# A-Kokolis/Hermes

Measured on AMD Instinct MI355X. Metric: replicated KVS ops/s (reads+writes committed), higher is better.
Workload: dtype u8

## Files before the change

hermes_amd/csrc/hkv_batch_dev.h:

```cpp
#pragma once
#include <hip/hip_runtime.h>

#include <type_traits>

#include "hkv_exec.h"
#include "hkv_internal.h"
#include "hkv_table_dev.h"

namespace hkv {

constexpr uint32_t kNone = 0xFFFFFFFFu;
enum : uint8_t { kStDone = 0, kStCommit = 1, kStPend = 2, kStDefer = 3 };
enum { kCtrFbM = 1, kCtrFbL = 2, kCtrDefer = 3 };

struct BatchArgs {
    uint8_t *elems;
    const int32_t *counts;
    const int32_t *offsets;
    const uint8_t *index;
    uint8_t *log;
    uint8_t *rw;
    int32_t *ns_idx;
    unsigned long long *fw;
    unsigned long long *fx, *fy;
    unsigned long long *ft;
    uint32_t fw_mask;
    uint32_t *ent;
    uint8_t *st;
    uint32_t *pf;
    uint8_t *shadow;
    unsigned long long *mem;
    uint32_t *fbl;
    uint32_t *ctr;
    unsigned int *error_flags;
    Geometry g;
    int64_t n;
    int64_t rw_stride;
    int32_t stride;
    int32_t esz;
    int32_t type;
    uint32_t rtag0;
    uint8_t ltag;
    int32_t rounds;
    int32_t inv_direct;
    int32_t ack_direct;
    uint8_t g_membership;
    uint8_t w_ack_init;
    int32_t *node_suspected;
    int32_t n_batches;
    const uint8_t *host_src;
    uint8_t *host_dst;
    uint8_t *dev_region;
    uint64_t region_bytes;
    uint32_t *done_flag;
    uint32_t done_value;
    unsigned long long *prof;
    const SmallBatch *hdr;
    uint8_t *state_out;
    const uint8_t *opc;
    const uint8_t *patch;
    uint16_t *fk;
    uint64_t *hx;
    uint8_t *rws;
    const uint8_t *rwo;
    int32_t n_rows, skip_row;
    int64_t row_stride;
    int32_t dbg;
    int32_t check_unique;
    uint8_t *ack_out;
    uint32_t ack_out_size;
    uint8_t *line;
};

enum class Engine : uint8_t {
    kSmall,
    kLocalDirect,
    kRows,
    kUniqueLds64,
    kUniqueLdsBig,
    kUniqueInPlace,
    kValsOnePass,
    kRoundsAckDirect,
    kRoundsInvDirect,
    kRoundsSlab,
    kRoundsInPlace,
};
enum class Patches : uint8_t {
    kNone,
    kApplyFirst,
    kByEngine,
    kInResolve,
};
constexpr uint32_t kPirMaxValue = 320;
constexpr uint32_t kWaveWordsMaxValue = 8 * 62;
static_assert(kPirMaxValue <= kWaveWordsMaxValue, "wave_value_copies_n ignores VCopy::fill: handle it there first");
struct BatchPlan {
    int refuse;
    Engine engine;
    Patches patches;
    int sv;
    int rmax, ch;
    int slab_threads;
    int64_t lookup_head;
    bool big;
    bool mixed;
    bool inv_direct, ack_direct;
    bool ack_out;
    bool state_out, opc;
    bool fk;
    bool rw_mirrors;
    bool node_suspected;
    bool il;
    bool inline_instance;
};

int launch_small(const BatchArgs &a, const BatchPlan &p, hipStream_t s);
int launch_local(const BatchArgs &a, const BatchPlan &p, hipStream_t s);

template <class F>
inline void with_sv(int sv, F &&f)
{
    if (sv == 31) f(std::integral_constant<int, 31>{});
    else if (sv == 287) f(std::integral_constant<int, 287>{});
    else f(std::integral_constant<int, 0>{});
}
template <class F>
inline void with_bool(bool b, F &&f)
{
    if (b) f(std::true_type{});
    else f(std::false_type{});
}

__device__ __forceinline__ Ctx make_ctx(const BatchArgs &a)
{
    Ctx c;
    c.g = a.g;
    c.g_membership = a.g_membership;
    c.w_ack_init = a.w_ack_init;
    c.rw = nullptr;
    c.rws = nullptr;
    c.rw_done = nullptr;
    c.vc = nullptr;
    return c;
}

__device__ __forceinline__ uint64_t phys_of(const BatchArgs &a, uint32_t e) { return (uint64_t)e * a.g.entry_unit; }
__device__ __forceinline__ uint8_t *entry_of(const BatchArgs &a, uint32_t e) { return a.log + phys_of(a, e); }

struct __attribute__((aligned(8))) U64x2 {
    uint64_t a, b;
};

template <int TYPE>
__device__ __forceinline__ uint8_t absorbing_state()
{
    return TYPE == kVals ? kValid : kWrite;
}

template <int TYPE>
__device__ __forceinline__ Meta after_first(const BatchArgs &a, const Meta &m0, uint32_t f, int f_is_put)
{
    Meta m1 = m0;
    m_set_state(m1, absorbing_state<TYPE>());
    if (TYPE != kLocal || a.g.skew == 0) return m1;
    uint8_t foc = f_is_put ? (uint8_t)kOpPut : a.elems[(int64_t)f * a.esz + 8];
    if (a.hx && !f_is_put) {
        const uint64_t pb = *reinterpret_cast<const uint64_t *>(a.patch + (int64_t)f * 16 + 8);
        if ((pb >> 48) & 0xFFu) foc = (uint8_t)pb;
    }
    if (foc != kOpGet) {
        m1.ver += 2;
        m_set_cid(m1, (uint8_t)a.g.machine_id);
    } else {
        m_set_state(m1, kReplay);
    }
    return m1;
}

__device__ __forceinline__ int32_t batch_of(const BatchArgs &a, int64_t i, int64_t &start)
{
    if (!a.offsets) {
        const int32_t b = (int32_t)(i / a.stride);
        start = (int64_t)b * a.stride;
        return b;
    }
    int lo = 0, hi = a.n_batches - 1;
    while (lo < hi) {
        const int mid = (lo + hi + 1) >> 1;
        if (a.offsets[mid] <= i) lo = mid; else hi = mid - 1;
    }
    start = a.offsets[lo];
    return lo;
}

__device__ __forceinline__ void elem_at(const BatchArgs &a, uint32_t i, uint8_t *&x, uint8_t &idx, Ctx &c)
{
    c.rw = nullptr;
    c.rws = nullptr;
    idx = 0;
    if (a.rw || !a.offsets) {
        int64_t start;
        const int32_t b = batch_of(a, i, start);
        idx = (uint8_t)(i - start);
        c.rw = a.rw ? a.rw + (int64_t)b * a.rw_stride : nullptr;
        c.rws = a.rws ? a.rws + (int64_t)b * (a.rw_stride / a.g.op_size) : nullptr;
        c.rwo = a.rwo ? a.rwo + (int64_t)b * (a.rw_stride / a.g.op_size) : nullptr;
    }
    x = a.elems + (int64_t)i * a.esz;
}

__device__ __forceinline__ void note_state(const BatchArgs &a, int64_t i, const uint8_t *x)
{
    if (a.state_out) a.state_out[i] = x[9];
}

__device__ __forceinline__ uint32_t fw_index(const BatchArgs &a, uint64_t phys)
{
    return (uint32_t)(((phys >> 6) * 0x9E3779B1ull) & a.fw_mask);
}
__device__ __forceinline__ unsigned long long *fw_of(const BatchArgs &a, uint32_t e) { return a.fw + fw_index(a, phys_of(a, e)); }

__device__ __forceinline__ uint32_t first_cand(unsigned long long f, uint32_t rtag)
{
    return (uint32_t)(f >> 32) == ~rtag ? (uint32_t)f : kNone;
}

__device__ __forceinline__ void offer(unsigned long long *f, uint32_t rtag, uint32_t i)
{
    const unsigned long long v = ((unsigned long long)(~rtag) << 32) | i;
    if (v < __hip_atomic_load(f, __ATOMIC_RELAXED, __HIP_MEMORY_SCOPE_AGENT)) atomicMin(f, v);
}

__device__ __forceinline__ uint8_t *shadow_of(const BatchArgs &a, uint32_t i)
{
    return a.shadow + (size_t)i * a.g.entry_size;
}

__device__ __forceinline__ void copy_entry(uint8_t *dst, const uint8_t *src, uint32_t bytes)
{
    struct __attribute__((aligned(8))) W16 {
        uint64_t a, b;
    };
    uint32_t o = 0;
    for (; o + 16 <= bytes; o += 16) *reinterpret_cast<W16 *>(dst + o) = *reinterpret_cast<const W16 *>(src + o);
    if (o < bytes) *reinterpret_cast<uint64_t *>(dst + o) = *reinterpret_cast<const uint64_t *>(src + o);
}

template <int TYPE, int SV>
__device__ __forceinline__ void apply_to_shadow(const BatchArgs &a, uint8_t *x, uint32_t i, const uint8_t *src)
{
    uint8_t *sh = shadow_of(a, i);
    Meta m;
    meta_load(src, m);
    if (SV == 31) {
        const uint4 *s4 = reinterpret_cast<const uint4 *>(src);
        uint4 *d4 = reinterpret_cast<uint4 *>(sh);
        const uint4 w0 = s4[0], w1 = s4[1], w2 = s4[2], w3 = s4[3];
        d4[0] = w0;
        d4[1] = w1;
        d4[2] = w2;
        d4[3] = w3;
    } else {
        copy_entry(sh, src, a.g.entry_size);
    }
    Ctx c = make_ctx(a);
    uint8_t *xg;
    uint8_t idx;
    elem_at(a, i, xg, idx, c);
    if (x) dispatch<SV>(TYPE, x, sh, idx, m, c);
    else dispatch<SV>(TYPE, xg, sh, idx, m, c);
    meta_store(sh, m);
}

__device__ __forceinline__ bool patch_valid(uint64_t pb) { return ((pb >> 48) & 0xFFu) != 0; }

__device__ __forceinline__ bool in_count(const BatchArgs &a, uint32_t i)
{
    if (!a.counts) return true;
    const uint32_t b = i / (uint32_t)a.stride;
    return (int32_t)(i - b * (uint32_t)a.stride) < a.counts[b];
}

__device__ __forceinline__ uint64_t line_key_meta(const uint4 &ln, Meta &m)
{
    const uint64_t ek = (uint64_t)(uint32_t)__shfl((int)ln.z, 0, 4) | ((uint64_t)(uint32_t)__shfl((int)ln.w, 0, 4) << 32);
    m.w4 = (uint32_t)__shfl((int)ln.x, 1, 4);
    m.w5 = (uint32_t)__shfl((int)ln.y, 1, 4);
    m.ver = (uint32_t)__shfl((int)ln.z, 1, 4);
    const uint32_t w7 = (uint32_t)__shfl((int)ln.w, 1, 4);
    const uint32_t b32 = (uint32_t)__shfl((int)ln.x, 2, 4) & 0xFFu;
    m.llw_cid = (uint8_t)w7;
    m.llw_ver = (w7 >> 8) | (b32 << 24);
    return ek;
}

constexpr int kLookupPair = 2;
template <int P = kLookupPair, bool IL = false, bool F = false>
__device__ __forceinline__ void lookup_core(const BatchArgs &a, const uint64_t *key, const bool *probe, int q,
                                            int gbase, bool *ok, uint64_t *phys, uint4 *ln, unsigned long long *fwv,
                                            uint8_t **home, bool *inl)
{
    uint4 v[P], ev[P];
#pragma unroll
    for (int k = 0; k < P; ++k) {
        if (IL) {
            const uint4 *l = line_words(a.line, bucket_of(a.g, key[k]));
            v[k] = probe[k] ? l[q] : make_uint4(0u, 0u, 0u, 0u);
            ev[k] = probe[k] ? l[4 + q] : make_uint4(0u, 0u, 0u, 0u);
        } else {
            v[k] = probe[k] ? bucket_words(a.index, bucket_of(a.g, key[k]))[q] : make_uint4(0u, 0u, 0u, 0u);
        }
    }
    bool il[P];
#pragma unroll
    for (int k = 0; k < P; ++k) {
        const uint64_t s0 = u64_of(v[k].x, v[k].y), s1 = u64_of(v[k].z, v[k].w);
        const uint32_t tag = key_tag(key[k]);
        const bool mt0 = probe[k] && (s0 & 1u) && ((uint32_t)(s0 >> 1) & 0x7FFFFFu) == tag;
        const bool mt1 = probe[k] && (s1 & 1u) && ((uint32_t)(s1 >> 1) & 0x7FFFFFu) == tag;
        const uint32_t g0 = (uint32_t)(__ballot(mt0) >> gbase) & 0xFu;
        const uint32_t g1 = (uint32_t)(__ballot(mt1) >> gbase) & 0xFu;
        uint32_t o = 0;
#pragma unroll
        for (int l = 0; l < 4; ++l) o |= ((g0 >> l) & 1u) << (2 * l) | ((g1 >> l) & 1u) << (2 * l + 1);
        const int first = o ? __ffs(o) - 1 : 0;
        const uint64_t raw = group_slot_word(slot_off_raw(s0), slot_off_raw(s1), first), off = off_of<IL>(raw);
        ok[k] = probe[k] && o && in_log_window(a.g, off);
        phys[k] = off & a.g.log_mask;
        il[k] = off_is_inline<IL>(raw) && ok[k];
    }
#pragma unroll
    for (int k = 0; k < P; ++k) {
        if (IL) {
            ln[k] = ev[k];
            if (!il[k]) ln[k] = ok[k] ? reinterpret_cast<const uint4 *>(a.log + phys[k])[q] : make_uint4(0u, 0u, 0u, 0u);
            if (home) home[k] = il[k] ? line_entry(a.line, a.g, key[k]) : a.log + phys[k];
            if (inl) inl[k] = il[k];
        } else {
            ln[k] = ok[k] ? reinterpret_cast<const uint4 *>(a.log + phys[k])[q] : make_uint4(0u, 0u, 0u, 0u);
            if (home) home[k] = a.log + phys[k];
            if (inl) inl[k] = false;
        }
        if (F) fwv[k] = ok[k] && q == 0 ? a.fw[fw_index(a, phys[k])] : ~0ull;
    }
}

template <int P = kLookupPair, bool IL = false>
__device__ __forceinline__ void lookup_pair(const BatchArgs &a, const uint64_t *key, const bool *probe, int q,
                                            int gbase, bool *ok, uint64_t *phys, uint4 *ln, uint8_t **home = nullptr,
                                            bool *inl = nullptr)
{
    lookup_core<P, IL, false>(a, key, probe, q, gbase, ok, phys, ln, nullptr, home, inl);
}

template <int P, bool IL = false>
__device__ __forceinline__ void lookup_pair_f(const BatchArgs &a, const uint64_t *key, const bool *probe, int q,
                                              int gbase, bool *ok, uint64_t *phys, uint4 *ln, unsigned long long *fwv,
                                              uint8_t **home = nullptr, bool *inl = nullptr)
{
    lookup_core<P, IL, true>(a, key, probe, q, gbase, ok, phys, ln, fwv, home, inl);
}

}
```

hermes_amd/csrc/hkv_batch_local.hip:

```cpp
#include <hip/hip_runtime.h>

#include "hkv_batch_dev.h"

namespace hkv {

#ifdef HKV_DEBUG_MODES
#define HKV_DBG_ON(a, bit) (((a).dbg & (bit)) != 0)
#else
#define HKV_DBG_ON(a, bit) false
#endif

constexpr int kPreElems = 2048;
constexpr int kPreThreads = kPreElems / 4;
constexpr int kPreHead = 1024;
constexpr int kPreHash = 2048;

constexpr uint32_t kEntInline = 0x80000000u;
template <bool IL>
__device__ __forceinline__ uint32_t ent_id(uint32_t e) { return IL ? e & ~kEntInline : e; }
template <bool IL>
__device__ __forceinline__ uint8_t *entry_home(const BatchArgs &a, uint32_t e, uint64_t key)
{
    if (IL && (e & kEntInline)) return line_entry(a.line, a.g, key);
    return entry_of(a, ent_id<IL>(e));
}

__device__ __forceinline__ uint64_t elem_key(const BatchArgs &a, int64_t i)
{
    if (a.patch && a.patch[i * 16 + 14]) return *reinterpret_cast<const uint64_t *>(a.patch + i * 16);
    return *reinterpret_cast<const uint64_t *>(a.elems + i * a.esz);
}

__device__ __forceinline__ uint4 patch_chunk(uint4 w, int q, uint64_t pa, uint64_t pb)
{
    const uint32_t fill = (uint32_t)((pb >> 32) & 0xFFu) * 0x01010101u;
    const bool vfill = fill != 0, reset = ((pb >> 40) & 0xFFu) != 0;
    if (q == 0) {
        w.x = (uint32_t)pa;
        w.y = (uint32_t)(pa >> 32);
        w.z = (uint32_t)(pb & 0xFFu) | ((uint32_t)kNew << 8) | ((uint32_t)((pb >> 8) & 0xFFu) << 16) |
              (reset ? 0u : (w.z & 0xFF000000u));
        if (reset) w.w = 0;
    } else if (q == 1) {
        const uint32_t flags = (uint32_t)((pb >> 16) & 0xFFFFu);
        w.x = flags | (vfill ? (fill & 0xFFFF0000u) : (w.x & 0xFFFF0000u));
        if (vfill) w.y = w.z = w.w = fill;
    } else if (q == 2) {
        if (vfill) w.x = w.y = w.z = w.w = fill;
    } else if (vfill) {
        w.x = (w.x & 0xFFFFFF00u) | (fill & 0xFFu);
    }
    return w;
}

__device__ __forceinline__ uint32_t pre_slot(uint64_t key)
{
    return (uint32_t)((key * 0x9E3779B97F4A7C15ull) >> (64 - __builtin_ctz(kPreHash))) & (kPreHash - 1);
}

__device__ __forceinline__ bool pre_insert(uint64_t *hk, uint32_t *hv, uint64_t key, uint32_t i, bool &created,
                                           uint32_t &slot)
{
    created = false;
    if (key == ~0ull) return false;
    uint32_t sl = pre_slot(key);
    for (int n = 0; n < kPreHash; ++n) {
        const unsigned long long old = atomicCAS((unsigned long long *)&hk[sl], ~0ull, key);
        if (old == ~0ull || old == key) {
            created = old == ~0ull;
            atomicMin(&hv[sl], i);
            slot = sl;
            return true;
        }
        sl = (sl + 1) & (kPreHash - 1);
    }
    return false;
}

__device__ __forceinline__ void pre_insert_key(uint64_t *hk, uint64_t key)
{
    if (key == ~0ull) return;
    uint32_t sl = pre_slot(key);
    for (int n = 0; n < kPreHash; ++n) {
        const unsigned long long old = atomicCAS((unsigned long long *)&hk[sl], ~0ull, key);
        if (old == ~0ull || old == key) return;
        sl = (sl + 1) & (kPreHash - 1);
    }
}

constexpr int kPrePair = 4;
template <bool IL = false>
__global__ __launch_bounds__(kPreThreads) void k_local_pre(BatchArgs a)
{
    constexpr int HEAD = kPreHead;
    __shared__ uint64_t hk[kPreHash], gk[kPreHash];
    __shared__ uint32_t hv[kPreHash];
    __shared__ uint32_t dl[kPreElems];
    __shared__ uint32_t nd;
    const int tid = threadIdx.x, q = tid & 3, gbase = (tid & 63) & ~3;
    if (tid == 0) {
        nd = 0;
        if (blockIdx.x == 0) a.ctr[kCtrDefer] = 0;
    }
    for (int j = tid; j < kPreHash; j += kPreThreads) {
        hk[j] = ~0ull;
        gk[j] = ~0ull;
        hv[j] = kNone;
    }
    if (HKV_DBG_ON(a, 8)) return;
    const int64_t i0 = (int64_t)blockIdx.x * kPreElems;
    const int64_t head_end = HKV_DBG_ON(a, 4) ? 0 : i0 < HEAD ? i0 : HEAD;
    constexpr int kOwnK = kPreElems / kPreThreads, kAllK = kOwnK + (HEAD + kPreThreads - 1) / kPreThreads;
    U64x2 h[kAllK];
    bool in[kAllK];
    uint8_t opm[kAllK];
    U64x2 pt[kAllK];
#pragma unroll
    for (int k = 0; k < kAllK; ++k) {
        const bool own = k < kOwnK;
        const int64_t i = own ? i0 + k * kPreThreads + tid : (int64_t)(k - kOwnK) * kPreThreads + tid;
        in[k] = i < a.n && (own || i < head_end);
        opm[k] = a.opc ? a.opc[in[k] ? i : 0] : (uint8_t)kOpPut;
    }
    if (a.patch) {
#pragma unroll
        for (int k = 0; k < kAllK; ++k) {
            const bool own = k < kOwnK;
            const int64_t i = own ? i0 + k * kPreThreads + tid : (int64_t)(k - kOwnK) * kPreThreads + tid;
            pt[k] = in[k] && opm[k] == kOpPut ? *reinterpret_cast<const U64x2 *>(a.patch + i * 16) : U64x2{0, 0};
        }
#pragma unroll
        for (int k = 0; k < kAllK; ++k) {
            const bool own = k < kOwnK;
            const int64_t i = own ? i0 + k * kPreThreads + tid : (int64_t)(k - kOwnK) * kPreThreads + tid;
            h[k] = *reinterpret_cast<const U64x2 *>(a.elems + (in[k] && opm[k] == kOpPut && !patch_valid(pt[k].b) ? i : 0) * 56);
        }
    } else {
#pragma unroll
        for (int k = 0; k < kAllK; ++k) {
            const bool own = k < kOwnK;
            const int64_t i = own ? i0 + k * kPreThreads + tid : (int64_t)(k - kOwnK) * kPreThreads + tid;
            h[k] = *reinterpret_cast<const U64x2 *>(a.elems + (in[k] && opm[k] == kOpPut ? i : 0) * 56);
            pt[k] = U64x2{0, 0};
        }
    }
#pragma unroll
    for (int k = 0; k < kAllK; ++k)
        if (patch_valid(pt[k].b)) {
            h[k].a = pt[k].a;
            h[k].b = (h[k].b & ~0xFFFFull) | (pt[k].b & 0xFFu) | ((uint64_t)kNew << 8);
        }
#pragma unroll
    for (int k = 0; k < kAllK; ++k) {
        const bool own = k < kOwnK;
        const int64_t i = own ? i0 + k * kPreThreads + tid : (int64_t)(k - kOwnK) * kPreThreads + tid;
        in[k] = in[k] && opm[k] == kOpPut && in_count(a, (uint32_t)i);
    }
    if (HKV_DBG_ON(a, 16)) {
        uint64_t acc = 0;
#pragma unroll
        for (int k = 0; k < kAllK; ++k) acc += h[k].a ^ h[k].b;
        if (acc == 0x1234567ull) a.ctr[7] = 1;
        return;
    }
    __syncthreads();
#pragma unroll
    for (int k = 0; k < kAllK; ++k) {
        const bool own = k < kOwnK;
        const uint32_t i = (uint32_t)(own ? i0 + k * kPreThreads + tid : (int64_t)(k - kOwnK) * kPreThreads + tid);
        const uint64_t key = h[k].a;
        if (!(in[k] && (uint8_t)h[k].b == kOpPut && !skip_elem_os(kLocal, kOpPut, (uint8_t)(h[k].b >> 8)))) continue;
        bool created;
        uint32_t sl;
        if (own) {
            const bool in_table = pre_insert(hk, hv, key, i, created, sl);
            if (!in_table || created) {
                dl[atomicAdd(&nd, 1u)] = in_table ? sl : ~i;
            }
        } else {
            pre_insert_key(gk, key);
        }
    }
    __syncthreads();
    const Ctx c = make_ctx(a);
    const uint64_t hput[2] = {0, (uint64_t)kOpPut};
    const uint32_t cnt = HKV_DBG_ON(a, 2) ? 0 : nd;
    for (uint32_t base = 0; base < cnt; base += (kPreThreads / 4) * kPrePair) {
        uint64_t key[kPrePair];
        bool probe[kPrePair], ok[kPrePair];
        uint32_t idx[kPrePair];
        uint64_t phys[kPrePair];
        uint4 ln[kPrePair];
#pragma unroll
        for (int k = 0; k < kPrePair; ++k) {
            const uint32_t j = base + k * (kPreThreads / 4) + (tid >> 2);
            probe[k] = j < cnt;
            const uint32_t d = probe[k] ? dl[j] : 0u;
            idx[k] = !probe[k] ? kNone : d < (uint32_t)kPreHash ? hv[d] : ~d;
            key[k] = !probe[k] ? 0 : d < (uint32_t)kPreHash ? hk[d] : elem_key(a, (int64_t)idx[k]);
            if (probe[k] && head_end > 0 && key[k] != ~0ull) {
                uint32_t sl = pre_slot(key[k]);
                for (int n = 0; n < kPreHash; ++n) {
                    const uint64_t g = gk[sl];
                    if (g == ~0ull) break;
                    if (g == key[k]) {
                        probe[k] = false;
                        break;
                    }
                    sl = (sl + 1) & (kPreHash - 1);
                }
            }
        }
        lookup_pair<kPrePair, IL>(a, key, probe, q, gbase, ok, phys, ln);
#pragma unroll
        for (int k = 0; k < kPrePair; ++k) {
            Meta m0;
            const uint64_t ek = line_key_meta(ln[k], m0);
            if (q != 0 || !ok[k] || ek != key[k]) continue;
            if (!would_mutate(kLocal, reinterpret_cast<const uint8_t *>(hput), m0, c) || HKV_DBG_ON(a, 1)) continue;
            atomicMin(a.fw + fw_index(a, phys[k]), ((unsigned long long)(~a.rtag0) << 32) | idx[k]);
        }
    }
}

__device__ __forceinline__ void local_resolve_nm(const BatchArgs &a, uint8_t *x, const uint8_t *ent, const Meta &m)
{
    const uint8_t oc = x[8], st = m_state(m);
    const bool obi_empty = m_obi(m) == kObiEmpty;
    bool mut = false;
    if (oc == kOpGet) {
        if (st == kValid) {
            copy_value<31>(x + kOpValueOff, ent + kEntryValueOff, 31);
            x[9] = kGetComplete;
            x[10] = (uint8_t)((m_val_len(m) >> a.g.shift) - kOpMetaSize);
        } else if (st == kInvalidWrite || st == kWrite || st == kReplay) {
            x[9] = kGetStall;
        } else {
            x[9] = kEmpty;
            if (st == kInvalid) {
                const uint8_t lw = m_lwid(m);
                if (lw < 8 && ((a.g_membership >> lw) & 1u)) x[9] = kGetStall;
                else mut = obi_empty;
            }
        }
        if (a.g.skew & kSkewReadComplete) hot_read_complete(x, m.ver, m_cid(m));
    } else if (oc == kOpPut) {
        mut = (st == kValid || st == kInvalid) && obi_empty;
        x[9] = kPutStall;
        if (a.g.skew & kSkewWriteCoalesce) {
            const uint32_t cv = m.ver & 0xFFFFu;
            uint32_t over = ld32(x + 12);
            if (st != kReplay && over == 0) {
                st32(x + 12, cv);
                over = cv;
            }
            if (over > 0 && over + 1u < cv) x[9] = kPutComplete;
        }
    }
    if (mut && a.error_flags) atomicOr(a.error_flags, 1u);
}

__device__ __forceinline__ void local_first_lds(const BatchArgs &a, uint8_t *x, uint32_t i, uint8_t *ent, Meta m)
{
    Ctx c = make_ctx(a);
    const uint8_t idx = (uint8_t)(i - i / (uint32_t)a.stride * (uint32_t)a.stride);
    if (x[8] == kOpGet) exec_read<31>(x, ent, idx, m, c);
    else if (x[8] == kOpPut) exec_write<31>(x, ent, idx, m, c);
    meta_store(ent, m);
}

constexpr int kLfWaves = 2;
template <bool IL = false>
__global__ __launch_bounds__(64 * kLfWaves) __attribute__((amdgpu_num_sgpr(80))) void k_local_fused(BatchArgs a)
{
    constexpr int P = 2, NW = kLfWaves;
    constexpr int E = 16 * P;
    constexpr int EB = E * NW;
    static_assert(EB == 64, "one wave resolves the block, one element per lane");
    __shared__ uint4 sops_b[EB * 4];
    __shared__ uint4 sln_b[EB * 4];
    __shared__ unsigned long long sfw_b[EB];
    __shared__ uint32_t sent_b[EB];
    __shared__ uint8_t sprb_b[EB];
    __shared__ uint8_t sfl[EB];
    __shared__ uint32_t sst[EB / 4], sstate[EB / 4];
    __shared__ uint32_t sdef[EB];
    __shared__ uint32_t ndef;
    const int w = threadIdx.x >> 6, tid = threadIdx.x & 63, q = tid & 3, gbase = tid & ~3;
    uint4 *sops = sops_b + w * E * 4, *sln = sln_b + w * E * 4;
    unsigned long long *sfw = sfw_b + w * E;
    uint32_t *sent = sent_b + w * E;
    uint8_t *sprb = sprb_b + w * E;
    const int64_t ib = (int64_t)blockIdx.x * EB, i0 = ib + (int64_t)w * E;
    if (threadIdx.x == 0) ndef = 0;
    uint64_t key[P];
    bool probe[P], ok[P], live[P];
    uint64_t phys[P];
    uint4 ln[P], op[P];
    int te[P];
#pragma unroll
    for (int k = 0; k < P; ++k) {
        te[k] = k * 16 + (tid >> 2);
        const int64_t i = i0 + te[k];
        live[k] = i < a.n;
        op[k] = make_uint4(0u, 0u, 0u, 0u);
        if (live[k]) {
            const uint8_t *xg = a.elems + i * 56 + 16 * q;
            U64x2 p{0, 0};
            if (a.patch) p = *reinterpret_cast<const U64x2 *>(a.patch + i * 16);
            if (q < 3) {
                op[k] = *reinterpret_cast<const uint4 *>(xg);
            } else {
                const uint64_t t = *reinterpret_cast<const uint64_t *>(xg);
                op[k].x = (uint32_t)t;
                op[k].y = (uint32_t)(t >> 32);
            }
            if (patch_valid(p.b)) op[k] = patch_chunk(op[k], q, p.a, p.b);
        }
        sops[te[k] * 4 + q] = op[k];
    }
#pragma unroll
    for (int k = 0; k < P; ++k) {
        key[k] = (uint64_t)(uint32_t)__shfl((int)op[k].x, 0, 4) | ((uint64_t)(uint32_t)__shfl((int)op[k].y, 0, 4) << 32);
        const uint32_t h0 = (uint32_t)__shfl((int)op[k].z, 0, 4);
        probe[k] = false;
        if (live[k] && !HKV_DBG_ON(a, 128))
            probe[k] = in_count(a, (uint32_t)(i0 + te[k])) && !skip_elem_os(kLocal, (uint8_t)h0, (uint8_t)(h0 >> 8));
    }
    unsigned long long fwv[P];
    bool inl[P];
    if (HKV_DBG_ON(a, 512)) {
        lookup_pair<P, IL>(a, key, probe, q, gbase, ok, phys, ln, nullptr, inl);
#pragma unroll
        for (int k = 0; k < P; ++k) fwv[k] = ~0ull;
    } else {
        lookup_pair_f<P, IL>(a, key, probe, q, gbase, ok, phys, ln, fwv, nullptr, inl);
    }
#pragma unroll
    for (int k = 0; k < P; ++k) {
        Meta m;
        const uint64_t ek = line_key_meta(ln[k], m);
        const bool hit = ok[k] && ek == key[k];
        const unsigned long long f = hit && m_state(m) != kInvalid && q == 0 ? fwv[k] : ~0ull;
        if (hit) sln[te[k] * 4 + q] = ln[k];
        if (q == 0) {
            sfw[te[k]] = f;
            sent[te[k]] = hit ? (uint32_t)(phys[k] / a.g.entry_unit) | (IL && inl[k] ? kEntInline : 0u) : kNone;
            sprb[te[k]] = probe[k];
        }
    }
    __syncthreads();
    if (__builtin_amdgcn_readfirstlane(w) == 0 && !HKV_DBG_ON(a, 64)) {
        const int64_t i = ib + tid;
        uint8_t st = kStDone;
        if (i < a.n) {
            uint8_t *x = reinterpret_cast<uint8_t *>(&sops_b[tid * 4]);
            uint8_t *ent = reinterpret_cast<uint8_t *>(&sln_b[tid * 4]);
            const uint32_t e = sent_b[tid];
            const bool prb = sprb_b[tid] != 0;
            if (e != kNone) {
                Meta m;
                meta_load(ent, m);
                Ctx c = make_ctx(a);
                const bool wm = would_mutate(kLocal, x, m, c);
                if (m_state(m) == kInvalid) {
                    if (wm) {
                        const uint64_t ph = phys_of(a, ent_id<IL>(e));
                        offer(a.fw + fw_index(a, ph), a.rtag0, (uint32_t)i);
                        if ((uint8_t)(m.w5 >> 16) != a.ltag)
                            entry_home<IL>(a, e, *reinterpret_cast<const uint64_t *>(x))[kEntryMetaOff + 4] = a.ltag;
                    }
                    st = kStDefer;
                    sdef[atomicAdd(&ndef, 1u)] = (uint32_t)i;
                } else {
                    const uint32_t f = first_cand(sfw_b[tid], a.rtag0);
                    if (wm && (f == kNone || f > (uint32_t)i) && a.error_flags) atomicOr(a.error_flags, 4u);
                    if ((uint32_t)i == f) {
                        local_first_lds(a, x, (uint32_t)i, ent, m);
                        st = kStCommit;
                    } else {
                        local_resolve_nm(a, x, ent, f != kNone && (uint32_t)i > f ? after_first<kLocal>(a, m, f, 1) : m);
                    }
                }
            } else if (prb) {
                x[9] = kMiss;
            }
            if (a.opc && prb && x[8] == kOpPut && a.opc[i] != kOpPut && a.error_flags) atomicOr(a.error_flags, 8u);
            if (!HKV_DBG_ON(a, 1024)) a.ent[i] = e;
            reinterpret_cast<uint8_t *>(sst)[tid] = st;
            reinterpret_cast<uint8_t *>(sstate)[tid] = x[9];
        }
        const unsigned long long fm = __ballot(st == kStCommit);
        if (fm && !HKV_DBG_ON(a, 1024)) {
            if (st == kStCommit) sfl[__popcll(fm & ((1ull << tid) - 1ull))] = (uint8_t)tid;
            __threadfence_block();
            const int nf = __popcll(fm);
            for (int j = tid >> 2; j < nf; j += 16) {
                const int t = sfl[j];
                reinterpret_cast<uint4 *>(shadow_of(a, (uint32_t)(ib + t)))[q] = sln_b[t * 4 + q];
            }
        }
    }
    __syncthreads();
    if (!HKV_DBG_ON(a, 1024) && !HKV_DBG_ON(a, 64)) {
        if (ib + EB <= a.n && ((uintptr_t)a.state_out & 3) == 0) {
            if ((int)threadIdx.x < EB / 4) {
                reinterpret_cast<uint32_t *>(a.st + ib)[threadIdx.x] = sst[threadIdx.x];
                if (a.state_out) reinterpret_cast<uint32_t *>(a.state_out + ib)[threadIdx.x] = sstate[threadIdx.x];
            }
        } else if ((int)threadIdx.x < EB && ib + threadIdx.x < a.n) {
            a.st[ib + threadIdx.x] = reinterpret_cast<const uint8_t *>(sst)[threadIdx.x];
            if (a.state_out) a.state_out[ib + threadIdx.x] = reinterpret_cast<const uint8_t *>(sstate)[threadIdx.x];
        }
    }
    if (ndef && threadIdx.x == 0) {
        const uint32_t base = atomicAdd(&a.ctr[kCtrDefer], ndef);
        for (uint32_t j = 0; j < ndef; ++j) a.fbl[base + j] = sdef[j];
    }
#pragma unroll
    for (int k = 0; k < P; ++k) {
        if (!live[k] || HKV_DBG_ON(a, 256)) continue;
        uint8_t *xg = a.elems + (i0 + te[k]) * 56 + 16 * q;
        const uint4 v = sops[te[k] * 4 + q];
        if (q < 3) *reinterpret_cast<uint4 *>(xg) = v;
        else *reinterpret_cast<uint64_t *>(xg) = (uint64_t)v.x | ((uint64_t)v.y << 32);
    }
}

template <bool IL = false>
__global__ __launch_bounds__(256) void k_local_deferred(BatchArgs a)
{
    const uint32_t nd = a.ctr[kCtrDefer];
    for (uint32_t j = blockIdx.x * 256u + threadIdx.x; j < nd; j += gridDim.x * 256u) {
        const uint32_t i = a.fbl[j];
        const uint32_t e = a.ent[i];
        uint8_t *xg;
        uint8_t idx;
        Ctx c = make_ctx(a);
        elem_at(a, i, xg, idx, c);
        uint8_t *entry = IL ? entry_home<IL>(a, e, *reinterpret_cast<const uint64_t *>(xg)) : entry_of(a, e);
        Meta m;
        meta_load(entry, m);
        const uint32_t f = first_cand(*fw_of(a, ent_id<IL>(e)), a.rtag0);
        uint8_t st = kStDone;
        if (f == kNone || i < f) {
            Meta tm = m;
            dispatch<31>(kLocal, xg, entry, idx, tm, c);
            if (a.error_flags && !meta_equal(tm, m)) atomicOr(a.error_flags, 1u);
        } else if (i == f) {
            apply_to_shadow<kLocal, 31>(a, nullptr, i, entry);
            st = kStCommit;
        } else {
            const Meta m1 = after_first<kLocal>(a, m, f, 0);
            Meta tm = m1;
            dispatch<31>(kLocal, xg, entry, idx, tm, c);
            if (a.error_flags && !meta_equal(tm, m1)) atomicOr(a.error_flags, 1u);
        }
        a.st[i] = st;
        note_state(a, i, xg);
    }
}

constexpr int kCwElems = 1024;
template <bool IL = false>
__global__ __launch_bounds__(256) void k_commit_w(BatchArgs a)
{
    __shared__ uint32_t lst[4][kCwElems];
    const int lane = threadIdx.x & 63, w = threadIdx.x >> 6;
    const int64_t e0 = ((int64_t)blockIdx.x * 4 + w) * kCwElems + 16 * lane;
    uint32_t m = 0;
    if (e0 + 16 <= a.n) {
        const uint4 s4 = *reinterpret_cast<const uint4 *>(a.st + e0);
        const uint32_t sw[4] = {s4.x, s4.y, s4.z, s4.w};
#pragma unroll
        for (int b = 0; b < 16; ++b)
            if (((sw[b >> 2] >> (8 * (b & 3))) & 0xFFu) == kStCommit) m |= 1u << b;
    } else {
        for (int b = 0; b < 16; ++b)
            if (e0 + b < a.n && a.st[e0 + b] == kStCommit) m |= 1u << b;
    }
    const uint32_t c = __popc(m);
    uint32_t incl = c;
#pragma unroll
    for (int d = 1; d < 64; d <<= 1) {
        const uint32_t v = (uint32_t)__shfl_up((int)incl, d, 64);
        if (lane >= d) incl += v;
    }
    const uint32_t total = (uint32_t)__shfl((int)incl, 63, 64);
    for (uint32_t pos = incl - c; m; m &= m - 1) lst[w][pos++] = (uint32_t)e0 + (uint32_t)(__ffs(m) - 1);
    __syncthreads();
    const int q = lane & 3;
    for (uint32_t j = (uint32_t)(lane >> 2); j < total; j += 16) {
        const uint32_t i = lst[w][j];
        const uint4 v = reinterpret_cast<const uint4 *>(shadow_of(a, i))[q];
        if (IL) {
            const uint64_t key = (uint64_t)(uint32_t)__shfl((int)v.z, 0, 4) | ((uint64_t)(uint32_t)__shfl((int)v.w, 0, 4) << 32);
            reinterpret_cast<uint4 *>(entry_home<IL>(a, a.ent[i], key))[q] = v;
        } else {
            reinterpret_cast<uint4 *>(entry_of(a, a.ent[i]))[q] = v;
        }
    }
}

template <bool IL>
static void launch_local_il(const BatchArgs &a, hipStream_t s)
{
    const int64_t n = a.n;
    const dim3 pgrid((unsigned)((n + kPreElems - 1) / kPreElems));
    const dim3 fgrid((unsigned)((n + 32 * kLfWaves - 1) / (32 * kLfWaves)));
    hipLaunchKernelGGL(k_local_pre<IL>, pgrid, dim3(kPreThreads), 0, s, a);
    hipLaunchKernelGGL(k_local_fused<IL>, fgrid, dim3(64 * kLfWaves), 0, s, a);
    hipLaunchKernelGGL(k_local_deferred<IL>, dim3(128u), dim3(256), 0, s, a);
    hipLaunchKernelGGL(k_commit_w<IL>, dim3((unsigned)((n + 4 * kCwElems - 1) / (4 * kCwElems))), dim3(256), 0, s, a);
}

int launch_local(const BatchArgs &a, const BatchPlan &p, hipStream_t s)
{
    if (p.il) launch_local_il<true>(a, s);
    else launch_local_il<false>(a, s);
    return hipGetLastError() == hipSuccess ? 0 : -3;
}

}
```

Measured before the change: 5.005 billion.

## Compact commit lists per block and route deferred commits via a separate list

The fused kernel no longer writes a per-element state byte and entry id. Instead each 64-element block packs its first-writer shadows and entry ids densely at the front of its slot range, writes a per-block commit count, and places deferred elements at the back of the range. The commit kernel then reads one count per block instead of scanning a byte per element, and commits deferred first-writers from an atomically appended list stored in the mem buffer. It also keeps several shadow loads in flight per lane. This cuts global writes and reads of per-element state, at the cost of more atomics, reuse of the pf/mem buffers as scratch, and a changed meaning for the st array that other readers may rely on.

```diff
diff --git a/hermes_amd/csrc/hkv_batch_dev.h b/hermes_amd/csrc/hkv_batch_dev.h
--- a/hermes_amd/csrc/hkv_batch_dev.h
+++ b/hermes_amd/csrc/hkv_batch_dev.h
@@ -11,7 +11,7 @@
 
 constexpr uint32_t kNone = 0xFFFFFFFFu;
 enum : uint8_t { kStDone = 0, kStCommit = 1, kStPend = 2, kStDefer = 3 };
-enum { kCtrFbM = 1, kCtrFbL = 2, kCtrDefer = 3 };
+enum { kCtrFbM = 1, kCtrFbL = 2, kCtrDefer = 3, kCtrDefCommit = 4 };
 
 struct BatchArgs {
     uint8_t *elems;
@@ -247,9 +247,9 @@
 }
 
 template <int TYPE, int SV>
-__device__ __forceinline__ void apply_to_shadow(const BatchArgs &a, uint8_t *x, uint32_t i, const uint8_t *src)
-{
-    uint8_t *sh = shadow_of(a, i);
+__device__ __forceinline__ void apply_to_shadow_at(const BatchArgs &a, uint8_t *x, uint32_t i, const uint8_t *src,
+                                                   uint8_t *sh)
+{
     Meta m;
     meta_load(src, m);
     if (SV == 31) {
@@ -270,6 +270,11 @@
     if (x) dispatch<SV>(TYPE, x, sh, idx, m, c);
     else dispatch<SV>(TYPE, xg, sh, idx, m, c);
     meta_store(sh, m);
+}
+template <int TYPE, int SV>
+__device__ __forceinline__ void apply_to_shadow(const BatchArgs &a, uint8_t *x, uint32_t i, const uint8_t *src)
+{
+    apply_to_shadow_at<TYPE, SV>(a, x, i, src, shadow_of(a, i));
 }
 
 __device__ __forceinline__ bool patch_valid(uint64_t pb) { return ((pb >> 48) & 0xFFu) != 0; }
diff --git a/hermes_amd/csrc/hkv_batch_local.hip b/hermes_amd/csrc/hkv_batch_local.hip
--- a/hermes_amd/csrc/hkv_batch_local.hip
+++ b/hermes_amd/csrc/hkv_batch_local.hip
@@ -100,7 +100,7 @@
     const int tid = threadIdx.x, q = tid & 3, gbase = (tid & 63) & ~3;
     if (tid == 0) {
         nd = 0;
-        if (blockIdx.x == 0) a.ctr[kCtrDefer] = 0;
+        if (blockIdx.x == 0) a.ctr[kCtrDefer] = a.ctr[kCtrDefCommit] = 0;
     }
     for (int j = tid; j < kPreHash; j += kPreThreads) {
         hk[j] = ~0ull;
@@ -270,6 +270,12 @@
 }
 
 constexpr int kLfWaves = 2;
+constexpr int kLfElems = 32 * kLfWaves;
+__device__ __forceinline__ uint32_t defer_slot(const BatchArgs &a, int64_t ib, uint32_t j)
+{
+    const int64_t live = a.n - ib < kLfElems ? a.n - ib : kLfElems;
+    return (uint32_t)(ib + live - 1 - j);
+}
 template <bool IL = false>
 __global__ __launch_bounds__(64 * kLfWaves) __attribute__((amdgpu_num_sgpr(80))) void k_local_fused(BatchArgs a)
 {
@@ -283,7 +289,7 @@
     __shared__ uint32_t sent_b[EB];
     __shared__ uint8_t sprb_b[EB];
     __shared__ uint8_t sfl[EB];
-    __shared__ uint32_t sst[EB / 4], sstate[EB / 4];
+    __shared__ uint32_t sstate[EB / 4];
     __shared__ uint32_t sdef[EB];
     __shared__ uint32_t ndef;
     const int w = threadIdx.x >> 6, tid = threadIdx.x & 63, q = tid & 3, gbase = tid & ~3;
@@ -350,9 +356,11 @@
         }
     }
     __syncthreads();
-    if (__builtin_amdgcn_readfirstlane(w) == 0 && !HKV_DBG_ON(a, 64)) {
+    if (__builtin_amdgcn_readfirstlane(w) == 0 && HKV_DBG_ON(a, 64)) {
+        if (tid == 0) a.st[blockIdx.x] = 0;
+    } else if (__builtin_amdgcn_readfirstlane(w) == 0) {
         const int64_t i = ib + tid;
-        uint8_t st = kStDone;
+        bool first = false;
         if (i < a.n) {
             uint8_t *x = reinterpret_cast<uint8_t *>(&sops_b[tid * 4]);
             uint8_t *ent = reinterpret_cast<uint8_t *>(&sln_b[tid * 4]);
@@ -370,14 +378,15 @@
                         if ((uint8_t)(m.w5 >> 16) != a.ltag)
                             entry_home<IL>(a, e, *reinterpret_cast<const uint64_t *>(x))[kEntryMetaOff + 4] = a.ltag;
                     }
-                    st = kStDefer;
-                    sdef[atomicAdd(&ndef, 1u)] = (uint32_t)i;
+                    const uint32_t dj = atomicAdd(&ndef, 1u);
+                    sdef[dj] = (uint32_t)i;
+                    if (!HKV_DBG_ON(a, 1024)) a.ent[defer_slot(a, ib, dj)] = e;
                 } else {
                     const uint32_t f = first_cand(sfw_b[tid], a.rtag0);
                     if (wm && (f == kNone || f > (uint32_t)i) && a.error_flags) atomicOr(a.error_flags, 4u);
                     if ((uint32_t)i == f) {
                         local_first_lds(a, x, (uint32_t)i, ent, m);
-                        st = kStCommit;
+                        first = true;
                     } else {
                         local_resolve_nm(a, x, ent, f != kNone && (uint32_t)i > f ? after_first<kLocal>(a, m, f, 1) : m);
                     }
@@ -386,36 +395,36 @@
                 x[9] = kMiss;
             }
             if (a.opc && prb && x[8] == kOpPut && a.opc[i] != kOpPut && a.error_flags) atomicOr(a.error_flags, 8u);
-            if (!HKV_DBG_ON(a, 1024)) a.ent[i] = e;
-            reinterpret_cast<uint8_t *>(sst)[tid] = st;
             reinterpret_cast<uint8_t *>(sstate)[tid] = x[9];
         }
-        const unsigned long long fm = __ballot(st == kStCommit);
-        if (fm && !HKV_DBG_ON(a, 1024)) {
-            if (st == kStCommit) sfl[__popcll(fm & ((1ull << tid) - 1ull))] = (uint8_t)tid;
-            __threadfence_block();
+        const unsigned long long fm = __ballot(first);
+        if (!HKV_DBG_ON(a, 1024)) {
             const int nf = __popcll(fm);
-            for (int j = tid >> 2; j < nf; j += 16) {
-                const int t = sfl[j];
-                reinterpret_cast<uint4 *>(shadow_of(a, (uint32_t)(ib + t)))[q] = sln_b[t * 4 + q];
-            }
+            if (fm) {
+                if (first) sfl[__popcll(fm & ((1ull << tid) - 1ull))] = (uint8_t)tid;
+                __threadfence_block();
+                if (tid < nf) a.ent[ib + tid] = sent_b[sfl[tid]];
+                for (int j = tid >> 2; j < nf; j += 16)
+                    reinterpret_cast<uint4 *>(shadow_of(a, (uint32_t)(ib + j)))[q] = sln_b[sfl[j] * 4 + q];
+            }
+            if (tid == 0) a.st[blockIdx.x] = (uint8_t)nf;
         }
     }
     __syncthreads();
-    if (!HKV_DBG_ON(a, 1024) && !HKV_DBG_ON(a, 64)) {
+    if (!HKV_DBG_ON(a, 1024) && !HKV_DBG_ON(a, 64) && a.state_out) {
         if (ib + EB <= a.n && ((uintptr_t)a.state_out & 3) == 0) {
-            if ((int)threadIdx.x < EB / 4) {
-                reinterpret_cast<uint32_t *>(a.st + ib)[threadIdx.x] = sst[threadIdx.x];
-                if (a.state_out) reinterpret_cast<uint32_t *>(a.state_out + ib)[threadIdx.x] = sstate[threadIdx.x];
-            }
+            if ((int)threadIdx.x < EB / 4)
+                reinterpret_cast<uint32_t *>(a.state_out + ib)[threadIdx.x] = sstate[threadIdx.x];
         } else if ((int)threadIdx.x < EB && ib + threadIdx.x < a.n) {
-            a.st[ib + threadIdx.x] = reinterpret_cast<const uint8_t *>(sst)[threadIdx.x];
-            if (a.state_out) a.state_out[ib + threadIdx.x] = reinterpret_cast<const uint8_t *>(sstate)[threadIdx.x];
-        }
-    }
-    if (ndef && threadIdx.x == 0) {
+            a.state_out[ib + threadIdx.x] = reinterpret_cast<const uint8_t *>(sstate)[threadIdx.x];
+        }
+    }
+    if (ndef && threadIdx.x == 0 && !HKV_DBG_ON(a, 1024)) {
         const uint32_t base = atomicAdd(&a.ctr[kCtrDefer], ndef);
-        for (uint32_t j = 0; j < ndef; ++j) a.fbl[base + j] = sdef[j];
+        for (uint32_t j = 0; j < ndef; ++j) {
+            a.fbl[base + j] = sdef[j];
+            a.pf[base + j] = defer_slot(a, ib, j);
+        }
     }
 #pragma unroll
     for (int k = 0; k < P; ++k) {
@@ -432,8 +441,8 @@
 {
     const uint32_t nd = a.ctr[kCtrDefer];
     for (uint32_t j = blockIdx.x * 256u + threadIdx.x; j < nd; j += gridDim.x * 256u) {
-        const uint32_t i = a.fbl[j];
-        const uint32_t e = a.ent[i];
+        const uint32_t i = a.fbl[j], s = a.pf[j];
+        const uint32_t e = a.ent[s];
         uint8_t *xg;
         uint8_t idx;
         Ctx c = make_ctx(a);
@@ -442,44 +451,55 @@
         Meta m;
         meta_load(entry, m);
         const uint32_t f = first_cand(*fw_of(a, ent_id<IL>(e)), a.rtag0);
-        uint8_t st = kStDone;
         if (f == kNone || i < f) {
             Meta tm = m;
             dispatch<31>(kLocal, xg, entry, idx, tm, c);
             if (a.error_flags && !meta_equal(tm, m)) atomicOr(a.error_flags, 1u);
         } else if (i == f) {
-            apply_to_shadow<kLocal, 31>(a, nullptr, i, entry);
-            st = kStCommit;
+            apply_to_shadow_at<kLocal, 31>(a, nullptr, i, entry, shadow_of(a, s));
+            reinterpret_cast<uint32_t *>(a.mem)[atomicAdd(&a.ctr[kCtrDefCommit], 1u)] = s;
         } else {
             const Meta m1 = after_first<kLocal>(a, m, f, 0);
             Meta tm = m1;
             dispatch<31>(kLocal, xg, entry, idx, tm, c);
             if (a.error_flags && !meta_equal(tm, m1)) atomicOr(a.error_flags, 1u);
         }
-        a.st[i] = st;
         note_state(a, i, xg);
     }
 }
 
-constexpr int kCwElems = 1024;
+constexpr int kCwBlocks = 16;
+constexpr int kCwWaves = 64 / kCwBlocks > 4 ? 4 : 64 / kCwBlocks;
+constexpr int kCwFlight = 4;
+
+template <bool IL>
+__device__ __forceinline__ void commit_images(const BatchArgs &a, const uint32_t *slot, const bool *ok, int q)
+{
+    uint4 v[kCwFlight];
+    uint32_t e[kCwFlight];
+#pragma unroll
+    for (int k = 0; k < kCwFlight; ++k) {
+        v[k] = ok[k] ? reinterpret_cast<const uint4 *>(shadow_of(a, slot[k]))[q] : make_uint4(0u, 0u, 0u, 0u);
+        e[k] = ok[k] ? a.ent[slot[k]] : kNone;
+    }
+#pragma unroll
+    for (int k = 0; k < kCwFlight; ++k) {
+        const uint64_t key = (uint64_t)(uint32_t)__shfl((int)v[k].z, 0, 4) | ((uint64_t)(uint32_t)__shfl((int)v[k].w, 0, 4) << 32);
+        if (ok[k]) reinterpret_cast<uint4 *>(entry_home<IL>(a, e[k], key))[q] = v[k];
+    }
+}
+
 template <bool IL = false>
-__global__ __launch_bounds__(256) void k_commit_w(BatchArgs a)
-{
-    __shared__ uint32_t lst[4][kCwElems];
-    const int lane = threadIdx.x & 63, w = threadIdx.x >> 6;
-    const int64_t e0 = ((int64_t)blockIdx.x * 4 + w) * kCwElems + 16 * lane;
-    uint32_t m = 0;
-    if (e0 + 16 <= a.n) {
-        const uint4 s4 = *reinterpret_cast<const uint4 *>(a.st + e0);
-        const uint32_t sw[4] = {s4.x, s4.y, s4.z, s4.w};
-#pragma unroll
-        for (int b = 0; b < 16; ++b)
-            if (((sw[b >> 2] >> (8 * (b & 3))) & 0xFFu) == kStCommit) m |= 1u << b;
-    } else {
-        for (int b = 0; b < 16; ++b)
-            if (e0 + b < a.n && a.st[e0 + b] == kStCommit) m |= 1u << b;
-    }
-    const uint32_t c = __popc(m);
+__global__ __launch_bounds__(64 * kCwWaves) void k_commit_w(BatchArgs a)
+{
+    __shared__ uint32_t lst[kCwWaves][kCwBlocks * kLfElems];
+    if (HKV_DBG_ON(a, 1024)) return;
+    const int lane = threadIdx.x & 63, w = threadIdx.x >> 6, q = lane & 3, g = lane >> 2;
+    const int64_t b = ((int64_t)blockIdx.x * kCwWaves + w) * kCwBlocks + lane;
+    const int64_t left = a.n - b * kLfElems;
+    const uint32_t live = left <= 0 ? 0u : left < kLfElems ? (uint32_t)left : (uint32_t)kLfElems;
+    uint32_t c = lane < kCwBlocks && live ? a.st[b] : 0u;
+    if (c > live) c = live;
     uint32_t incl = c;
 #pragma unroll
     for (int d = 1; d < 64; d <<= 1) {
@@ -487,18 +507,32 @@
         if (lane >= d) incl += v;
     }
     const uint32_t total = (uint32_t)__shfl((int)incl, 63, 64);
-    for (uint32_t pos = incl - c; m; m &= m - 1) lst[w][pos++] = (uint32_t)e0 + (uint32_t)(__ffs(m) - 1);
+    for (uint32_t j = 0; j < c; ++j) lst[w][incl - c + j] = (uint32_t)(b * kLfElems) + j;
     __syncthreads();
-    const int q = lane & 3;
-    for (uint32_t j = (uint32_t)(lane >> 2); j < total; j += 16) {
-        const uint32_t i = lst[w][j];
-        const uint4 v = reinterpret_cast<const uint4 *>(shadow_of(a, i))[q];
-        if (IL) {
-            const uint64_t key = (uint64_t)(uint32_t)__shfl((int)v.z, 0, 4) | ((uint64_t)(uint32_t)__shfl((int)v.w, 0, 4) << 32);
-            reinterpret_cast<uint4 *>(entry_home<IL>(a, a.ent[i], key))[q] = v;
-        } else {
-            reinterpret_cast<uint4 *>(entry_of(a, a.ent[i]))[q] = v;
-        }
+    for (uint32_t base = 0; base < total; base += 16 * kCwFlight) {
+        uint32_t slot[kCwFlight];
+        bool ok[kCwFlight];
+#pragma unroll
+        for (int k = 0; k < kCwFlight; ++k) {
+            const uint32_t j = base + 16 * k + g;
+            ok[k] = j < total;
+            slot[k] = ok[k] ? lst[w][j] : 0u;
+        }
+        commit_images<IL>(a, slot, ok, q);
+    }
+    const uint32_t ndc = a.ctr[kCtrDefCommit];
+    const uint32_t *dl = reinterpret_cast<const uint32_t *>(a.mem);
+    const uint32_t groups = gridDim.x * kCwWaves * 16u;
+    for (uint32_t base = (blockIdx.x * kCwWaves + w) * 16u + g; base < ndc; base += groups * kCwFlight) {
+        uint32_t slot[kCwFlight];
+        bool ok[kCwFlight];
+#pragma unroll
+        for (int k = 0; k < kCwFlight; ++k) {
+            const uint32_t j = base + groups * k;
+            ok[k] = j < ndc;
+            slot[k] = ok[k] ? dl[j] : 0u;
+        }
+        commit_images<IL>(a, slot, ok, q);
     }
 }
 
@@ -507,11 +541,12 @@
 {
     const int64_t n = a.n;
     const dim3 pgrid((unsigned)((n + kPreElems - 1) / kPreElems));
-    const dim3 fgrid((unsigned)((n + 32 * kLfWaves - 1) / (32 * kLfWaves)));
+    const int64_t nblk = (n + kLfElems - 1) / kLfElems;
+    const dim3 fgrid((unsigned)nblk), cgrid((unsigned)((nblk + kCwWaves * kCwBlocks - 1) / (kCwWaves * kCwBlocks)));
     hipLaunchKernelGGL(k_local_pre<IL>, pgrid, dim3(kPreThreads), 0, s, a);
     hipLaunchKernelGGL(k_local_fused<IL>, fgrid, dim3(64 * kLfWaves), 0, s, a);
     hipLaunchKernelGGL(k_local_deferred<IL>, dim3(128u), dim3(256), 0, s, a);
-    hipLaunchKernelGGL(k_commit_w<IL>, dim3((unsigned)((n + 4 * kCwElems - 1) / (4 * kCwElems))), dim3(256), 0, s, a);
+    hipLaunchKernelGGL(k_commit_w<IL>, cgrid, dim3(64 * kCwWaves), 0, s, a);
 }
 
 int launch_local(const BatchArgs &a, const BatchPlan &p, hipStream_t s)
```

New measurement: 5.052 billion (median of 6 runs). About the same (+0.9%).
